# gauravchak/two_tower_models

Hardware: AMD Instinct MI355X
Metric: user-item pairs/sec (in-batch softmax train step: fwd + zero_grad + bwd + dense-exact Adam) (higher is better)
Workload: dtype f32

## Files before the change

### include/tt_hotpath.h

```cpp
#ifndef TT_HOTPATH_H
#define TT_HOTPATH_H

#include <stdint.h>

#ifdef __cplusplus
extern "C" {
#endif

#define TT_ABI_VERSION 6

#define TT_E_BADARG (-1)
#define TT_E_WORKSPACE (-2)
#define TT_E_UNSUPPORTED (-3)

typedef void* tt_stream_t;

int tt_abi_version(void);
const char* tt_last_error_string(void);

int tt_profile_enable(int on);
int tt_profile_read(const char* kernel, double* total_ms, int64_t* launches);
int tt_profile_filter(const char* kernels);
int tt_profile_pause(int paused);

// ... 192 lines not shown
} tt_adam_stash_job;
typedef struct {
  float *W, *M, *V;
  int64_t n_rows, dim;
  const tt_grad_sources* src;
  int64_t n_ids;
  const int32_t *sorted_ids, *perm, *seg_begin, *n_unique;
  void* side;
  int64_t side_bytes;
} tt_adam_finish_job;
int tt_adam_begin_ids(double* hyper, float* tab, int64_t tab_steps, const tt_adam_stash_job* jobs, int32_t n_jobs,
                      tt_stream_t stream);
int tt_adam_tables_finish(const tt_adam_finish_job* jobs, int32_t n_jobs, const double* hyper, tt_stream_t stream);
int tt_adam_begin_ids_planes(double* hyper, float* tab, int64_t tab_steps, const tt_adam_stash_job* jobs, int32_t n_jobs,
                             int32_t planes, tt_stream_t stream);

int tt_stream_create_low_priority(void** out_stream);
int tt_stream_destroy(void* stream);

int tt_adam_advance_tab(double* hyper, float* tab, int64_t tab_steps, tt_stream_t stream);
int tt_adam_rows_catchup(float* W, float* M, float* V, int64_t n_rows, int64_t dim, const int64_t* ids,
                         int64_t n_ids, int32_t* last_step, const double* hyper, const float* tab,
                         int64_t tab_steps, tt_stream_t stream);
int tt_adam_table_lazy(float* W, float* M, float* V, int64_t n_rows, int64_t dim, const double* hyper,
                       const tt_grad_sources* src , int64_t n_ids, const int32_t* sorted_ids,
                       const int32_t* perm, const int32_t* seg_begin, const int32_t* n_unique, void* ws,
                       int64_t ws_bytes, int32_t* last_step, const float* tab, int64_t tab_steps,
                       tt_stream_t stream);
int tt_adam_table_flush(float* W, float* M, float* V, int64_t n_rows, int64_t dim, int32_t* last_step,
                        const double* hyper, const float* tab, int64_t tab_steps, tt_stream_t stream);
// ... 161 lines not shown
```

### two_tower_models_amd/_native.py

```python
from __future__ import annotations

import ctypes as C
import os
from typing import Optional

import torch

_PKG = os.path.dirname(os.path.abspath(__file__))
LIB_PATH = os.path.join(_PKG, "lib", "libtt_hotpath.so")

TT_GEMM_NT, TT_GEMM_NN, TT_GEMM_TN = 0, 1, 2
TT_EPI_NONE, TT_EPI_RELU, TT_EPI_RELU_MASK = 0, 1, 2
TT_F32, TT_BF16, TT_F16X2 = 0, 1, 2
TT_E_BADARG, TT_E_WORKSPACE, TT_E_UNSUPPORTED = -1, -2, -3
TT_DEBIAS_COMBINED, TT_DEBIAS_POSITION, TT_DEBIAS_USER = 0, 1, 2
TT_COMM_ID_BYTES = 128
TT_COMM_F32, TT_COMM_I32, TT_COMM_I64, TT_COMM_U8 = 0, 1, 2, 3
TT_COMM_SUM, TT_COMM_MAX = 0, 1
TT_MAX_GRAD_SOURCES = 4
ABI_VERSION = 6

_vp, _i64, _i32, _int = C.c_void_p, C.c_int64, C.c_int32, C.c_int


class GradSources(C.Structure):

    _fields_ = [
        ("rows", _vp * TT_MAX_GRAD_SOURCES),
        ("ld", _i64 * TT_MAX_GRAD_SOURCES),
        ("first", _i64 * (TT_MAX_GRAD_SOURCES + 1)),
        ("n_sources", _i32),
    ]


class AdamTensor(C.Structure):

    _fields_ = [("p", _vp), ("g", _vp), ("m", _vp), ("v", _vp), ("n", _i64)]


class AdamStashJob(C.Structure):

    _fields_ = [("W", _vp), ("M", _vp), ("V", _vp), ("n_rows", _i64), ("dim", _i64), ("ids", _vp), ("n_ids", _i64),
                ("side", _vp), ("side_bytes", _i64)]


class AdamFinishJob(C.Structure):

    _fields_ = [("W", _vp), ("M", _vp), ("V", _vp), ("n_rows", _i64), ("dim", _i64), ("src", C.POINTER(GradSources)),
                ("n_ids", _i64), ("sorted_ids", _vp), ("perm", _vp), ("seg_begin", _vp), ("n_unique", _vp), ("side", _vp),
                ("side_bytes", _i64)]


# ... 94 lines not shown
    "tt_rowgrad_workspace_bytes": (_i64, [_i64]),
    "tt_rowgrad_plan": (_int, [_vp, _i64, _i64, _vp, _vp, _vp, _vp, _vp, _vp, _i64, _vp]),
    "tt_rowgrad_dense": (_int, [C.POINTER(GradSources), _i64, _i64, _vp, _vp, _vp, _vp, _vp, _vp]),
    "tt_adam_advance": (_int, [_vp, _vp]),
    "tt_adam_table_workspace_bytes": (_i64, [_i64, _i64]),
    "tt_adam_table": (_int, [_vp, _vp, _vp, _i64, _i64, _vp, C.POINTER(GradSources), _i64, _vp, _vp, _vp,
                             _vp, _vp, _i64, _vp]),
    "tt_adam_table_stash": (_int, [_vp, _vp, _vp, _i64, _i64, _i64, _vp, _vp, _vp, _vp, _vp, _i64, _vp]),
    "tt_adam_table_stash_ids": (_int, [_vp, _vp, _vp, _i64, _i64, _vp, _i64, _vp, _i64, _vp]),
    "tt_adam_table_sweep": (_int, [_vp, _vp, _vp, _i64, _i64, _vp, _vp]),
    "tt_adam_tables_sweep": (_int, [C.POINTER(AdamTensor), _i32, _vp, _i32, _vp]),
    "tt_adam_marks_words": (_i64, [_i64]),
    "tt_adam_marked_supported": (_int, [_i64]),
    "tt_adam_mark_rows": (_int, [_vp, _i64, _i64, _vp, _i64, _vp]),
    "tt_adam_tables_sweep_marked": (_int, [C.POINTER(AdamTensor), C.POINTER(_i64), C.POINTER(_vp), _i32, _vp, _i32, _vp]),
    "tt_adam_table_finish": (_int, [_vp, _vp, _vp, _i64, _i64, _vp, C.POINTER(GradSources), _i64, _vp, _vp, _vp,
                                    _vp, _vp, _i64, _vp]),
    "tt_adam_advance_tab": (_int, [_vp, _vp, _i64, _vp]),
    "tt_adam_rows_catchup": (_int, [_vp, _vp, _vp, _i64, _i64, _vp, _i64, _vp, _vp, _vp, _i64, _vp]),
    "tt_adam_table_lazy": (_int, [_vp, _vp, _vp, _i64, _i64, _vp, C.POINTER(GradSources), _i64, _vp, _vp, _vp, _vp,
                                  _vp, _i64, _vp, _vp, _i64, _vp]),
    "tt_adam_table_flush": (_int, [_vp, _vp, _vp, _i64, _i64, _vp, _vp, _vp, _i64, _vp]),
    "tt_stream_create_low_priority": (_int, [C.POINTER(_vp)]),
    "tt_stream_destroy": (_int, [_vp]),
    "tt_adam_dense": (_int, [C.POINTER(AdamTensor), _i32, _vp, _vp]),
    "tt_pack_grads": (_int, [C.POINTER(AdamTensor), _i32, _vp]),
    "tt_copy_buffers": (_int, [C.POINTER(AdamTensor), _i32, _vp]),
    "tt_hist_embed_pool": (_int, [_vp, _i64, _i64, _vp, _i64, _i64, _vp, _vp, _vp, _i64, _vp, _vp]),
    "tt_hist_dx_pool_bwd": (_int, [_vp, _vp, _i64, _i64, _i64, _vp, _i64, _vp, _vp]),
    "tt_hist_pool_bwd": (_int, [_vp, _i64, _i64, _i64, _vp, _i64, _vp]),
# ... 214 lines not shown
```

### two_tower_models_amd/csrc/adam.hip

```cpp
#include <stdlib.h>

#include "common.hpp"

namespace tt {

constexpr int SWEEP_MAX_TABLES_DECL = 4;

constexpr int SWEEP_DEFAULT_PERSIST = 3;

struct AdamConst {
  float one_minus_b1, b2, one_minus_b2, eps, neg_step_size, inv_bc2_sqrt;
};

__device__ __forceinline__ AdamConst load_hyper(const double* __restrict__ h) {
  AdamConst c;
  c.one_minus_b1 = (float)(1.0 - h[1]);
  c.b2 = (float)h[2];
  c.one_minus_b2 = (float)(1.0 - h[2]);
  c.eps = (float)h[3];
  c.neg_step_size = (float)(-h[5]);
  c.inv_bc2_sqrt = (float)(1.0 / h[6]);
  return c;
}

// ... 20 lines not shown
  al = e - (ah - p);
}
__device__ __forceinline__ double pow_steps(double b, double step) {
  double rh = 1.0, rl = 0.0, bh = b, bl = 0.0;
  for (unsigned long long e = (unsigned long long)step; e; e >>= 1) {
    if (e & 1) dd_mul(rh, rl, bh, bl);
    dd_mul(bh, bl, bh, bl);
  }
  return rh;
}
__device__ __forceinline__ void step_consts_from_doubles(double lr, double b1, double b2, double step,
                                                         double& h5, double& h6) {
  h5 = lr / (1.0 - pow_steps(b1, step));
  h6 = sqrt(1.0 - pow_steps(b2, step));
}
__global__ void adam_advance_kernel(double* h, float* tab, int64_t tab_cap) {
  const double step = h[4] + 1.0;
  h[4] = step;
  step_consts_from_doubles(h[0], h[1], h[2], step, h[5], h[6]);
  const int64_t j = (int64_t)step;
  if (tab && j < tab_cap) {
    tab[2 * j] = (float)(-h[5]);
    tab[2 * j + 1] = (float)(1.0 / h[6]);
  }
}

__device__ __forceinline__ const float* source_row(const tt_grad_sources& s, int64_t pos) {
  int k = 0;
#pragma unroll
  for (int q = 1; q < TT_MAX_GRAD_SOURCES; ++q)
    if (q < s.n_sources && pos >= s.first[q]) k = q;
  return s.rows[k] + (pos - s.first[k]) * s.ld[k];
}

template <bool FROM_SIDE>
__global__ __launch_bounds__(256) void adam_touched_kernel(const float* __restrict__ W, const float* __restrict__ M,
                                                           const float* __restrict__ V, int64_t n_rows, int64_t dim,
                                                           const double* __restrict__ hyper, const tt_grad_sources src,
                                                           const int32_t* __restrict__ sorted_ids,
                                                           const int32_t* __restrict__ perm,
// ... 97 lines not shown

struct StashJobs {
  const float* W[SWEEP_MAX_TABLES_DECL];
  const float* M[SWEEP_MAX_TABLES_DECL];
  const float* V[SWEEP_MAX_TABLES_DECL];
  const int64_t* ids[SWEEP_MAX_TABLES_DECL];
  float* side[SWEEP_MAX_TABLES_DECL];
  int64_t n_rows[SWEEP_MAX_TABLES_DECL], dim[SWEEP_MAX_TABLES_DECL], n_ids[SWEEP_MAX_TABLES_DECL];
  unsigned first_block[SWEEP_MAX_TABLES_DECL + 1];
  int n;
};
__global__ __launch_bounds__(256) void adam_begin_ids_kernel(const StashJobs jobs, double* h, float* tab, int64_t tab_cap, int planes,
                                                             int advance) {
  const unsigned n_stash = jobs.first_block[jobs.n];
  if (blockIdx.x == n_stash) {
    if (threadIdx.x == 0 && advance) {
      const double step = h[4] + 1.0;
      h[4] = step;
      step_consts_from_doubles(h[0], h[1], h[2], step, h[5], h[6]);
      const int64_t j = (int64_t)step;
      if (tab && j < tab_cap) {
        tab[2 * j] = (float)(-h[5]);
        tab[2 * j + 1] = (float)(1.0 / h[6]);
      }
    }
    return;
  }
  int t = 0;
#pragma unroll
  for (int q = 1; q < SWEEP_MAX_TABLES_DECL; ++q)
    if (q < jobs.n && blockIdx.x >= jobs.first_block[q]) t = q;
  adam_stash_ids_body(jobs.W[t], jobs.M[t], jobs.V[t], jobs.n_rows[t], jobs.dim[t], jobs.ids[t], jobs.n_ids[t], jobs.side[t],
                      blockIdx.x - jobs.first_block[t], planes);
}

__global__ __launch_bounds__(256) void adam_writeback_kernel(float* __restrict__ W, float* __restrict__ M,
                                                             float* __restrict__ V, int64_t n_rows, int64_t dim,
                                                             const int32_t* __restrict__ sorted_ids,
                                                             const int32_t* __restrict__ seg_begin,
                                                             const int32_t* __restrict__ perm,
// ... 137 lines not shown
      ctr[1] = 0;
      __threadfence();
    }
  }
}

constexpr int SWEEP_MAX_TABLES = SWEEP_MAX_TABLES_DECL;
struct SweepTables {
  float4* W[SWEEP_MAX_TABLES];
  float4* M[SWEEP_MAX_TABLES];
  float4* V[SWEEP_MAX_TABLES];
  int64_t n4[SWEEP_MAX_TABLES];
  unsigned first_chunk[SWEEP_MAX_TABLES + 1];
  int n;
};
template <int ITERS, int UNR>
__global__ __launch_bounds__(256) void adam_sweep_tables_kernel(const SweepTables tabs, const double* __restrict__ hyper,
                                                                unsigned* __restrict__ ctr) {
  const AdamConst c = load_hyper(hyper);
  const unsigned n_chunks = tabs.first_chunk[tabs.n];
  __shared__ unsigned s_next[2];
  if (threadIdx.x == 0) s_next[0] = atomicAdd(&ctr[0], 1u);
  __syncthreads();
  unsigned ch = s_next[0];
  int par = 0;
  while (ch < n_chunks) {
    if (threadIdx.x == 0) s_next[par ^ 1] = atomicAdd(&ctr[0], 1u);
    int t = 0;
#pragma unroll
    for (int q = 1; q < SWEEP_MAX_TABLES; ++q)
      if (q < tabs.n && ch >= tabs.first_chunk[q]) t = q;
    float4* __restrict__ W = tabs.W[t];
    float4* __restrict__ M = tabs.M[t];
    float4* __restrict__ V = tabs.V[t];
    const int64_t n4 = tabs.n4[t];
    const int64_t base = (int64_t)(ch - tabs.first_chunk[t]) * (256 * ITERS) + threadIdx.x;
#pragma unroll UNR
    for (int k = 0; k < ITERS; ++k) {
      const int64_t i = base + (int64_t)k * 256;
      if (i >= n4) break;
      float4 p = sweep_load(W + i), m = sweep_load(M + i), v = sweep_load(V + i);
      adam_elem_zero_grad(p.x, m.x, v.x, c);
      adam_elem_zero_grad(p.y, m.y, v.y, c);
      adam_elem_zero_grad(p.z, m.z, v.z, c);
      adam_elem_zero_grad(p.w, m.w, v.w, c);
      sweep_store(p, W + i); sweep_store(m, M + i); sweep_store(v, V + i);
    }
    __syncthreads();
    par ^= 1;
    ch = s_next[par];
  }
  if (threadIdx.x == 0) {
    if (atomicAdd(&ctr[1], 1u) == gridDim.x - 1) {
      ctr[0] = 0;
      ctr[1] = 0;
      __threadfence();
    }
  }
}

struct SweepTablesMarked {
  SweepTables t;
  const unsigned* marks[SWEEP_MAX_TABLES];
  int sh[SWEEP_MAX_TABLES];
};
template <int ITERS, int PAIR>
__global__ __launch_bounds__(256) void adam_sweep_tables_marked_kernel(const SweepTablesMarked tm, const double* __restrict__ hyper,
                                                                       unsigned* __restrict__ ctr) {
  const AdamConst c = load_hyper(hyper);
  const unsigned n_chunks = tm.t.first_chunk[tm.t.n];
  __shared__ unsigned s_next[2];
  if (threadIdx.x == 0) s_next[0] = atomicAdd(&ctr[0], 1u);
  __syncthreads();
  unsigned ch = s_next[0];
  int par = 0;
  while (ch < n_chunks) {
    if (threadIdx.x == 0) s_next[par ^ 1] = atomicAdd(&ctr[0], 1u);
    const unsigned chu = __builtin_amdgcn_readfirstlane(ch);
    int t = 0;
#pragma unroll
    for (int q = 1; q < SWEEP_MAX_TABLES; ++q)
      if (q < tm.t.n && chu >= tm.t.first_chunk[q]) t = q;
    float4* __restrict__ W = tm.t.W[t];
    float4* __restrict__ M = tm.t.M[t];
    float4* __restrict__ V = tm.t.V[t];
    const int64_t n4 = tm.t.n4[t];
    const unsigned lc = chu - tm.t.first_chunk[t];
    const int sh = tm.sh[t];
    const int64_t r0 = (int64_t)lc * ((256 * ITERS) >> sh);
    const unsigned* __restrict__ mk = tm.marks[t];
    unsigned w0 = 0, w1 = 0, w2 = 0, w3 = 0;
    if (mk) {
      const unsigned* mw = mk + (r0 >> 5);
      w0 = mw[0]; w1 = mw[1]; w2 = mw[2]; w3 = mw[3];
    }
    const int64_t base = (int64_t)lc * (256 * ITERS) + threadIdx.x;
#pragma unroll
    for (int k = 0; k < ITERS; k += PAIR) {
      float4 p[PAIR], m[PAIR], v[PAIR];
      bool live[PAIR];
#pragma unroll
      for (int q = 0; q < PAIR; ++q) {
        const int64_t i = base + (int64_t)(k + q) * 256;
        const int64_t row = r0 + (((k + q) * 256 + (int)threadIdx.x) >> sh);
        const int wj = (int)((row >> 5) - (r0 >> 5));
        const unsigned word = wj == 0 ? w0 : wj == 1 ? w1 : wj == 2 ? w2 : w3;
        live[q] = i < n4 && !((word >> (row & 31)) & 1u);
      }
#pragma unroll
      for (int q = 0; q < PAIR; ++q) {
        const int64_t i = base + (int64_t)(k + q) * 256;
        if (live[q]) { p[q] = sweep_load(W + i); m[q] = sweep_load(M + i); v[q] = sweep_load(V + i); }
      }
#pragma unroll
      for (int q = 0; q < PAIR; ++q) {
        const int64_t i = base + (int64_t)(k + q) * 256;
        if (live[q]) {
          adam_elem_zero_grad(p[q].x, m[q].x, v[q].x, c);
          adam_elem_zero_grad(p[q].y, m[q].y, v[q].y, c);
          adam_elem_zero_grad(p[q].z, m[q].z, v[q].z, c);
          adam_elem_zero_grad(p[q].w, m[q].w, v[q].w, c);
          sweep_store(p[q], W + i); sweep_store(m[q], M + i); sweep_store(v[q], V + i);
        }
      }
    }
    __syncthreads();
    par ^= 1;
    ch = s_next[par];
  }
  if (threadIdx.x == 0) {
    if (atomicAdd(&ctr[1], 1u) == gridDim.x - 1) {
      ctr[0] = 0;
      ctr[1] = 0;
      __threadfence();
    }
  }
}

__global__ __launch_bounds__(256) void adam_mark_rows_kernel(const int64_t* __restrict__ ids, int64_t n_ids, int64_t n_rows,
                                                             unsigned* __restrict__ marks) {
  const int64_t i = (int64_t)blockIdx.x * 256 + threadIdx.x;
  if (i >= n_ids) return;
  const int64_t row = ids[i];
  if (row >= 0 && row < n_rows) atomicOr(&marks[row >> 5], 1u << (row & 31));
}

__global__ __launch_bounds__(256) void adam_sweep_scalar_kernel(float* __restrict__ W, float* __restrict__ M,
                                                                float* __restrict__ V, int64_t i0, int64_t n,
                                                                const double* __restrict__ hyper) {
  const AdamConst c = load_hyper(hyper);
  const int64_t stride = (int64_t)gridDim.x * blockDim.x;
  for (int64_t i = i0 + (int64_t)blockIdx.x * blockDim.x + threadIdx.x; i < n; i += stride) {
    float p = W[i], m = M[i], v = V[i];
    adam_elem_zero_grad(p, m, v, c);
    W[i] = p; M[i] = m; V[i] = v;
  }
}

__device__ __forceinline__ void replay_consts(AdamConst& c, const double* __restrict__ h, const float* __restrict__ tab,
// ... 350 lines not shown
  if (!ids || !marks) return fail_arg("tt_adam_mark_rows: null pointer");
  if (n_ids <= 0 || n_rows <= 0) return fail_arg("tt_adam_mark_rows: sizes");
  if (marks_words < tt_adam_marks_words(n_rows)) { set_error("tt_adam_mark_rows: bitmap of %lld words < %lld", (long long)marks_words, (long long)tt_adam_marks_words(n_rows)); return TT_E_WORKSPACE; }
  hipStream_t st = S(stream);
  hipError_t e = hipMemsetAsync(marks, 0, (size_t)marks_words * 4, st);
  if (e != hipSuccess) { set_error("tt_adam_mark_rows: hipMemsetAsync: %s", hipGetErrorString(e)); return (int)e; }
  adam_mark_rows_kernel<<<(unsigned)ceil_div(n_ids, 256), 256, 0, st>>>(ids, n_ids, n_rows, marks);
  return check_launch("adam_mark_rows_kernel");
}

extern "C" int tt_adam_marked_supported(int64_t dim) {
  if (dim < 32 || dim > 4096 || (dim & (dim - 1))) return 0;
  return 1;
}

extern "C" int tt_adam_tables_sweep_marked(const tt_adam_tensor* tables, const int64_t* dims, const uint32_t* const* marks,
                                           int32_t n_tables, const double* hyper, int32_t n_wgs, tt_stream_t stream) {
  if (!tables || !dims || !marks || !hyper) return fail_arg("tt_adam_tables_sweep_marked: null pointer");
  if (n_tables <= 0 || n_tables > SWEEP_MAX_TABLES) return fail_arg("tt_adam_tables_sweep_marked: 1..4 tables");
  SweepTablesMarked tm{};
  unsigned chunks = 0;
  for (int t = 0; t < n_tables; ++t) {
    const tt_adam_tensor& d = tables[t];
    if (!d.p || !d.m || !d.v || d.n <= 0) return fail_arg("tt_adam_tables_sweep_marked: descriptor");
    if (!tt_adam_marked_supported(dims[t]) || d.n % dims[t]) return fail_arg("tt_adam_tables_sweep_marked: dim must be a power of two in [32, 4096]");
    if ((reinterpret_cast<uintptr_t>(d.p) | reinterpret_cast<uintptr_t>(d.m) | reinterpret_cast<uintptr_t>(d.v)) & 15)
      return fail_arg("tt_adam_tables_sweep_marked: 16-byte aligned tables");
    tm.t.W[t] = reinterpret_cast<float4*>(d.p); tm.t.M[t] = reinterpret_cast<float4*>(d.m); tm.t.V[t] = reinterpret_cast<float4*>(d.v);
    tm.t.n4[t] = d.n / 4;
    tm.t.first_chunk[t] = chunks;
    const int64_t c = ceil_div(d.n / 4, 256 * 4);
    if (c + chunks >= (1ll << 32)) return fail_arg("tt_adam_tables_sweep_marked: too many chunks");
    chunks += (unsigned)c;
    tm.marks[t] = marks[t];
    int sh = 0;
    while ((4ll << sh) < dims[t]) ++sh;
    tm.sh[t] = sh;
  }
  tm.t.first_chunk[n_tables] = chunks;
  tm.t.n = n_tables;
  static const int wgs_env = getenv("TT_SWEEP_WGS") ? atoi(getenv("TT_SWEEP_WGS")) : 0;
  const int want = getenv("TT_SWEEP_WGS") ? wgs_env : n_wgs;
  unsigned* ctr = reinterpret_cast<unsigned*>(const_cast<double*>(hyper) + 7);
  unsigned grid = (unsigned)(device_cu_count() * SWEEP_DEFAULT_PERSIST);
  if (want > 0 && (unsigned)want < grid) grid = (unsigned)want;
  hipStream_t st = S(stream);
  ProfScope prof("adam_sweep_kernel", st);
  adam_sweep_tables_marked_kernel<4, 2><<<grid, 256, 0, st>>>(tm, hyper, ctr);
  return check_launch("adam_sweep_tables_marked_kernel");
}

extern "C" int tt_stream_create_low_priority(void** out) {
  if (!out) return fail_arg("tt_stream_create_low_priority: null pointer");
  int least = 0, greatest = 0;
  hipError_t e = hipDeviceGetStreamPriorityRange(&least, &greatest);
  if (e != hipSuccess) { set_error("hipDeviceGetStreamPriorityRange: %s", hipGetErrorString(e)); return (int)e; }
  hipStream_t s;
  e = hipStreamCreateWithPriority(&s, hipStreamNonBlocking, least);
  if (e != hipSuccess) { set_error("hipStreamCreateWithPriority: %s", hipGetErrorString(e)); return (int)e; }
  *out = reinterpret_cast<void*>(s);
  return 0;
}
extern "C" int tt_stream_destroy(void* stream) {
  if (!stream) return 0;
// ... 230 lines not shown
```

### two_tower_models_amd/optim.py

```python
from __future__ import annotations

import ctypes as C
import os
import weakref
from typing import Dict, Iterable, List, Optional, Sequence

import torch

from . import _native as N
from . import ops
from .sweep_controller import GroupSweepController, SweepController


_RELEASE_AT_LOGITS = True
_TAB_MIN_STEPS = 1 << 16
_SPLIT_MIN_IDS = 65536
_MARK_ROWS = True
_HOLD_SWEEP = True


class _TableStep:

    __slots__ = ("plan", "side", "announced", "marked", "n_rows")

# ... 61 lines not shown
        self.capture_overlap = False
        self._sweep_ctl = (GroupSweepController(self._group_reduce(self._sharded[0]))
                           if self._sharded and self._sharded[0]._tt_shard.world > 1 else SweepController())
        self._plan_stream: Optional[torch.cuda.Stream] = None
        self._plan_done: Optional[torch.cuda.Event] = None
        self._plans_pending = False
        self._plan_ready: Optional[torch.cuda.Event] = None
        self._begun: Optional[Dict[torch.nn.Parameter, _TableStep]] = None
        self._sweep_done: Optional[torch.cuda.Event] = None
        self._side_bufs: Dict[int, torch.Tensor] = {}
        self._marks: Dict[int, torch.Tensor] = {}
        self._sweep_pending = None
        self._sweep_pending_marked = False
        self._sweep_events = None
        self._catchup_last: Dict[int, tuple] = {}

    def _init_state(self) -> None:
        dev = N.require_device(*self._params)
        g = self.param_groups[0]
        self._hyper = torch.tensor([g["lr"], g["betas"][0], g["betas"][1], g["eps"], 0.0, 0.0, 0.0, 0.0],
                                   dtype=torch.float64, device=dev)
        arena = bool(self._tables) and all(p.is_cuda for p in self._tables) and os.environ.get("TT_ADAM_NO_ARENA") is None
        in_arena = {id(p) for p in self._tables} if arena else set()
        for p in self._params:
            if p.dtype != torch.float32 or not p.is_contiguous():
                raise TypeError("DenseExactAdam needs contiguous fp32 parameters")
            st = self.state[p]
            for key in ("exp_avg", "exp_avg_sq"):
                if key not in st and id(p) in in_arena:
                    continue
# ... 156 lines not shown
    def state_dict(self):
        self.flush()
        sd = super().state_dict()
        step = torch.tensor(float(self.step_count))
        for st in sd["state"].values():
            st["step"] = step.clone()
        return sd

    def load_state_dict(self, state_dict) -> None:
        super().load_state_dict(state_dict)
        steps = {int(float(st["step"])) for st in self.state.values() if "step" in st}
        if len(steps) > 1:
            raise ValueError("DenseExactAdam needs one common step count for all parameters")
        self._resume_step = self._sweep_ctl.resume_step = steps.pop() if steps else 0
        self._begun = None
        self._ready = False

    def _advance_lazy(self) -> None:
        if (self._host_steps + 2 >= self._tab_steps and not self._tab_pinned
                and not torch.cuda.is_current_stream_capturing()):
            bigger = torch.zeros(4 * self._tab_steps, dtype=torch.float32, device=self._tab.device)
            bigger[: 2 * self._tab_steps].copy_(self._tab)
            self._tab, self._tab_steps = bigger, 2 * self._tab_steps
        N.check(N.load().tt_adam_advance_tab(self._hyper.data_ptr(), self._tab.data_ptr(), self._tab_steps,
                                             N.stream()), "tt_adam_advance_tab")
        self._host_steps += 1

    @property
    def step_count(self) -> int:
        if not self._ready:
# ... 1 lines not shown
        return int(self._hyper[4].item())

    def _side(self, p: torch.Tensor, nbytes: int) -> torch.Tensor:
        buf = self._side_bufs.get(id(p))
        if buf is None or buf.numel() < nbytes:
            buf = torch.empty(int(nbytes * 1.25) + 256, dtype=torch.uint8, device=p.device)
            self._side_bufs[id(p)] = buf
        return buf

    def _begin_overlapped(self, announced: Optional[Dict[int, Sequence[torch.Tensor]]] = None, hold_sweep: bool = False) -> None:
        lib = N.load()
        if not self._ready:
            self._init_state()
        hyper = self._hyper.data_ptr()
        capturing = torch.cuda.is_current_stream_capturing()
        ev_begin = None
        if capturing:
            self._sweep_ctl.record = None
        else:
            self._tune_sweep()
            ev_begin = torch.cuda.Event(enable_timing=True)
            ev_begin.record()
            self._sweep_ctl.began(ev_begin, self._host_steps + 1)
        if announced is None:
            N.check(lib.tt_adam_advance(hyper, N.stream()), "tt_adam_advance")
        self._host_steps += 1
        begun: Dict[torch.nn.Parameter, _TableStep] = {}
        stash_jobs = []
        todo = []
        for p in self._tables:
            blocks = announced.get(id(p)) if announced is not None else p._tt_lookups
            if not blocks:
                continue
            shard = getattr(p, "_tt_shard", None)
            n_rows = p.shape[0] if shard is None else shard.n_local
            if n_rows > 0:
                todo.append((p, blocks, n_rows))
        n_stashed = sum(sum(b.numel() for b in blocks) for _, blocks, _ in todo)
        split_planes = announced is not None and not capturing and 0 < len(todo) <= 4 and n_stashed >= _SPLIT_MIN_IDS
        marked = (split_planes and _MARK_ROWS and all(lib.tt_adam_marked_supported(p.shape[1]) for p, _, _ in todo)
                  and all((p.data_ptr() | self.state[p]["exp_avg"].data_ptr() | self.state[p]["exp_avg_sq"].data_ptr()) % 16 == 0
                          for p, _, _ in todo))
        for p, blocks, n_rows in todo:
            dim = p.shape[1]
            shard = getattr(p, "_tt_shard", None)
            st = self.state[p]
            plan = ops.RowPlan(blocks, n_rows + (1 if shard is not None else 0), slot=f"plan{id(p)}", defer=announced is not None)
            side = None if marked else self._side(p, lib.tt_adam_table_workspace_bytes(plan.n, dim))
            if marked:
                if shard is None:
                    p._tt_active = ops.ActiveMarks(plan.block_sizes)
            elif announced is not None:
                stash_jobs.append((p.data_ptr(), st["exp_avg"].data_ptr(), st["exp_avg_sq"].data_ptr(), n_rows, dim,
                                   plan.ids.data_ptr(), plan.n, side.data_ptr(), side.numel()))
                if shard is None:
                    p_plane = side[: plan.n * dim * 4].view(torch.float32).view(plan.n, dim)
                    p._tt_active = ops.ActiveStash(p_plane, plan.block_sizes)
            else:
                N.check(lib.tt_adam_table_stash(p.data_ptr(), st["exp_avg"].data_ptr(), st["exp_avg_sq"].data_ptr(),
                                                n_rows, dim, plan.n, plan.sorted_ids.data_ptr(), plan.perm.data_ptr(),
                                                plan.seg_begin.data_ptr(), plan.n_unique.data_ptr(), side.data_ptr(),
                                                side.numel(), N.stream()), "tt_adam_table_stash")
            begun[p] = _TableStep(plan, side, announced is not None, marked, n_rows)
        if marked:
            N.check(lib.tt_adam_advance(hyper, N.stream()), "tt_adam_advance")
        elif announced is not None:
            jobs = (N.AdamStashJob * max(len(stash_jobs), 1))()
            for i, j in enumerate(stash_jobs):
                (jobs[i].W, jobs[i].M, jobs[i].V, jobs[i].n_rows, jobs[i].dim, jobs[i].ids, jobs[i].n_ids, jobs[i].side,
                 jobs[i].side_bytes) = j
            if split_planes:
                N.check(lib.tt_adam_begin_ids_planes(hyper, None, 0, jobs, len(stash_jobs), 1, N.stream()), "tt_adam_begin_ids_planes")
            else:
                N.check(lib.tt_adam_begin_ids(hyper, None, 0, jobs, len(stash_jobs), N.stream()), "tt_adam_begin_ids")
        main = torch.cuda.current_stream()
        ready = torch.cuda.Event()
        ready.record(main)

# ... 36 lines not shown
                if mark_ptrs is not None:
                    dims = (C.c_int64 * len(begun))(*[p.shape[1] for p in begun])
                    N.check(lib.tt_adam_tables_sweep_marked(descs, dims, mark_ptrs, len(begun), hyper, self._sweep_wgs,
                                                            self._side_stream.cuda_stream), "tt_adam_tables_sweep_marked")
                else:
                    N.check(lib.tt_adam_tables_sweep(descs, len(begun), hyper, self._sweep_wgs, self._side_stream.cuda_stream),
                            "tt_adam_tables_sweep")
            self._sweep_done = torch.cuda.Event(enable_timing=not capturing)
            self._sweep_done.record(self._side_stream)
            if not capturing:
                self._sweep_ctl.swept(ev_s0, self._sweep_done)
            if self._sweep_events is not None and ev_s0 is not None and len(self._sweep_events) < 65536:
                self._sweep_events.append((ev_s0, self._sweep_done))

        self._sweep_done = None
        n_announced = sum(ts.plan.n for ts in begun.values()) if announced is not None else 0
        if _HOLD_SWEEP and announced is not None and not capturing and ((n_announced >= 65536 and not self._sharded) or hold_sweep):
            self._sweep_pending = launch_sweep
            self._sweep_pending_marked = marked
            self._hold_for_logits = bool(hold_sweep) and _RELEASE_AT_LOGITS
            if self._hold_for_logits:
                ops.held_sweeps.add(self)
        else:
            self._sweep_pending = None
            launch_sweep()
        self._plan_done = None
        self._plans_pending = announced is not None and bool(begun)
        self._plan_ready = ready if self._plans_pending else None
        self._begun = begun

    def keep_sweep_events(self, on: bool = True) -> None:
        self._sweep_events = [] if on else None

    def sweep_launch_ms(self):
        total, n = 0.0, 0
        for a, b in self._sweep_events or ():
            b.synchronize()
            total += a.elapsed_time(b)
            n += 1
        return total, n

    def held_sweep_is_marked(self) -> bool:
        return getattr(self, "_sweep_pending", None) is not None and bool(getattr(self, "_sweep_pending_marked", False))
# ... 120 lines not shown
    @staticmethod
    def _ordered_rows(p) -> List[torch.Tensor]:
        blocks = p._tt_rowgrads
        if len(blocks) != len(p._tt_lookups) or any(b.index is None for b in blocks):
            raise RuntimeError(
                "a table lookup of the last forward received no gradient (or more than one forward ran "
                "before zero_grad()); use DenseExactAdam(..., overlap_sweep=False) for this call pattern")
        return [b.rows for b in sorted(blocks, key=lambda b: b.index)]

    @torch.no_grad()
    def step(self, closure=None):
        if closure is not None:
            raise NotImplementedError("closure is not supported")
        if not self._ready:
            self._init_state()
        lib = N.load()
        hyper = self._hyper.data_ptr()
        if self._sharded and self._begun is None:
            raise RuntimeError("row-sharded tables: step() without a train_forward that announced its lookups (the models' "
                               "train_forward does; a custom forward must call model._announce_lookups first)")
        reduce = self._start_dense_allreduce() if self._sharded else None
        self.release_sweep()
        if self._begun is not None:
            self._launch_plans(side=False)
            torch.cuda.current_stream().wait_event(self._sweep_done)
            if self._plan_done is not None:
                torch.cuda.current_stream().wait_event(self._plan_done)
                self._plan_done = None
            if self._begun:
                jobs = (N.AdamFinishJob * len(self._begun))()
                for i, (p, ts) in enumerate(self._begun.items()):
                    st = self.state[p]
                    ts.plan.attach(self._ordered_rows(p))
                    j = jobs[i]
                    j.W, j.M, j.V = p.data_ptr(), st["exp_avg"].data_ptr(), st["exp_avg_sq"].data_ptr()
                    shard = getattr(p, "_tt_shard", None)
                    j.n_rows = p.shape[0] if shard is None else shard.n_local
                    j.dim, j.src, j.n_ids = p.shape[1], C.pointer(ts.plan.sources), ts.plan.n
                    j.sorted_ids, j.perm = ts.plan.sorted_ids.data_ptr(), ts.plan.perm.data_ptr()
                    j.seg_begin, j.n_unique = ts.plan.seg_begin.data_ptr(), ts.plan.n_unique.data_ptr()
                    j.side, j.side_bytes = (None, 0) if ts.marked else (ts.side.data_ptr(), ts.side.numel())
                N.check(lib.tt_adam_tables_finish(jobs, len(self._begun), hyper, N.stream()), "tt_adam_tables_finish")
            self._begun = None
            if self._sweep_ctl.record is not None:
                end = torch.cuda.Event(enable_timing=True)
                end.record()
                self._sweep_ctl.ended(end)
        elif self.lazy:
            if self._prefetch_done is not None:
                torch.cuda.current_stream().wait_event(self._prefetch_done)
                self._prefetch_done, self._prefetch_keep = None, None
            self._catchup_last.clear()
            self._advance_lazy()
            todo = []
            for p in self._tables:
                blocks = p._tt_rowgrads
                if p.grad is not None:
                    raise RuntimeError("embedding table received a dense gradient while in row-gradient mode")
                if not blocks:
                    continue
                if all(b.index is not None for b in blocks):
# ... 40 lines not shown
        if reduce is not None:
            self._finish_dense_allreduce(reduce, lib, hyper)
            return None
        live = [p for p in self._dense if p.grad is not None]
        if live:
            descs = (N.AdamTensor * len(live))()
            keep = []
            for i, p in enumerate(live):
                gr = p.grad if p.grad.is_contiguous() else p.grad.contiguous()
                keep.append(gr)
                st = self.state[p]
                descs[i].p, descs[i].g = p.data_ptr(), gr.data_ptr()
                descs[i].m, descs[i].v = st["exp_avg"].data_ptr(), st["exp_avg_sq"].data_ptr()
                descs[i].n = p.numel()
            N.check(lib.tt_adam_dense(descs, len(live), hyper, N.stream()), "tt_adam_dense")
        return None
```

Before: 1.514 million.

## Chain marked Adam table sweep on side stream across optimizer step boundary

Adds a chained mode in which a fused mark+advance kernel runs on a side stream, followed by a marked sweep that skips touched rows. The main stream no longer waits for the sweep before the table finish step; it only waits at the very end of step(). Double-buffered mark bitmaps are cleared a step ahead, and an alone-flag lets surplus sweep workgroups exit once the main stream reaches the end of step, so the sweep can overlap backward and dense Adam without keeping the whole GPU. This adds cross-stream ordering complexity and a possible race on marks and hyper state.

```diff
diff --git a/include/tt_hotpath.h b/include/tt_hotpath.h
--- a/include/tt_hotpath.h
+++ b/include/tt_hotpath.h
@@ -230,6 +230,17 @@
 int tt_adam_tables_finish(const tt_adam_finish_job* jobs, int32_t n_jobs, const double* hyper, tt_stream_t stream);
 int tt_adam_begin_ids_planes(double* hyper, float* tab, int64_t tab_steps, const tt_adam_stash_job* jobs, int32_t n_jobs,
                              int32_t planes, tt_stream_t stream);
+typedef struct {
+  const int64_t* ids;
+  int64_t n_ids, n_rows;
+  uint32_t* marks;
+  int64_t marks_words;
+} tt_adam_mark_job;
+int tt_adam_mark_advance(double* hyper, const tt_adam_mark_job* jobs , int32_t n_jobs, tt_stream_t stream);
+int tt_adam_tables_sweep_chained(const struct tt_adam_tensor_s* tables , const int64_t* dims ,
+                                 const uint32_t* const* marks , int32_t n_tables,
+                                 const double* hyper, int32_t n_wgs, int32_t alone_wgs, const uint32_t* alone_flag,
+                                 uint32_t tag, tt_stream_t stream);
 
 int tt_stream_create_low_priority(void** out_stream);
 int tt_stream_destroy(void* stream);
diff --git a/two_tower_models_amd/_native.py b/two_tower_models_amd/_native.py
--- a/two_tower_models_amd/_native.py
+++ b/two_tower_models_amd/_native.py
@@ -36,6 +36,11 @@
 class AdamTensor(C.Structure):
 
     _fields_ = [("p", _vp), ("g", _vp), ("m", _vp), ("v", _vp), ("n", _i64)]
+
+
+class AdamMarkJob(C.Structure):
+
+    _fields_ = [("ids", _vp), ("n_ids", _i64), ("n_rows", _i64), ("marks", _vp), ("marks_words", _i64)]
 
 
 class AdamStashJob(C.Structure):
@@ -160,6 +165,9 @@
     "tt_adam_marked_supported": (_int, [_i64]),
     "tt_adam_mark_rows": (_int, [_vp, _i64, _i64, _vp, _i64, _vp]),
     "tt_adam_tables_sweep_marked": (_int, [C.POINTER(AdamTensor), C.POINTER(_i64), C.POINTER(_vp), _i32, _vp, _i32, _vp]),
+    "tt_adam_mark_advance": (_int, [_vp, C.POINTER(AdamMarkJob), _i32, _vp]),
+    "tt_adam_tables_sweep_chained": (_int, [C.POINTER(AdamTensor), C.POINTER(_i64), C.POINTER(_vp), _i32, _vp, _i32, _i32, _vp,
+                                            C.c_uint32, _vp]),
     "tt_adam_table_finish": (_int, [_vp, _vp, _vp, _i64, _i64, _vp, C.POINTER(GradSources), _i64, _vp, _vp, _vp,
                                     _vp, _vp, _i64, _vp]),
     "tt_adam_advance_tab": (_int, [_vp, _vp, _i64, _vp]),
diff --git a/two_tower_models_amd/csrc/adam.hip b/two_tower_models_amd/csrc/adam.hip
--- a/two_tower_models_amd/csrc/adam.hip
+++ b/two_tower_models_amd/csrc/adam.hip
@@ -1,4 +1,6 @@
 #include <stdlib.h>
+
+#include <type_traits>
 
 #include "common.hpp"
 
@@ -58,7 +60,7 @@
   h5 = lr / (1.0 - pow_steps(b1, step));
   h6 = sqrt(1.0 - pow_steps(b2, step));
 }
-__global__ void adam_advance_kernel(double* h, float* tab, int64_t tab_cap) {
+__device__ __forceinline__ void advance_step(double* h, float* tab, int64_t tab_cap) {
   const double step = h[4] + 1.0;
   h[4] = step;
   step_consts_from_doubles(h[0], h[1], h[2], step, h[5], h[6]);
@@ -68,6 +70,7 @@
     tab[2 * j + 1] = (float)(1.0 / h[6]);
   }
 }
+__global__ void adam_advance_kernel(double* h, float* tab, int64_t tab_cap) { advance_step(h, tab, tab_cap); }
 
 __device__ __forceinline__ const float* source_row(const tt_grad_sources& s, int64_t pos) {
   int k = 0;
@@ -195,16 +198,7 @@
                                                              int advance) {
   const unsigned n_stash = jobs.first_block[jobs.n];
   if (blockIdx.x == n_stash) {
-    if (threadIdx.x == 0 && advance) {
-      const double step = h[4] + 1.0;
-      h[4] = step;
-      step_consts_from_doubles(h[0], h[1], h[2], step, h[5], h[6]);
-      const int64_t j = (int64_t)step;
-      if (tab && j < tab_cap) {
-        tab[2 * j] = (float)(-h[5]);
-        tab[2 * j + 1] = (float)(1.0 / h[6]);
-      }
-    }
+    if (threadIdx.x == 0 && advance) advance_step(h, tab, tab_cap);
     return;
   }
   int t = 0;
@@ -372,37 +366,69 @@
   unsigned first_chunk[SWEEP_MAX_TABLES + 1];
   int n;
 };
-template <int ITERS, int UNR>
-__global__ __launch_bounds__(256) void adam_sweep_tables_kernel(const SweepTables tabs, const double* __restrict__ hyper,
-                                                                unsigned* __restrict__ ctr) {
+struct SweepTablesMarked {
+  SweepTables t;
+  const unsigned* marks[SWEEP_MAX_TABLES];
+  int sh[SWEEP_MAX_TABLES];
+};
+struct SweepTablesChained {
+  SweepTablesMarked m;
+  const unsigned* alone_flag;
+  unsigned tag, alone_wgs;
+};
+constexpr unsigned SWEEP_NO_CHUNK = 0xffffffffu;
+__device__ __forceinline__ unsigned next_chunk_or_leave(const SweepTablesChained& a, unsigned* ctr) {
+  if (a.alone_flag && blockIdx.x >= a.alone_wgs &&
+      __hip_atomic_load(a.alone_flag, __ATOMIC_RELAXED, __HIP_MEMORY_SCOPE_AGENT) == a.tag)
+    return SWEEP_NO_CHUNK;
+  return atomicAdd(&ctr[0], 1u);
+}
+template <int ITERS, int PAIR>
+__device__ __forceinline__ void sweep_chunk_marked(const SweepTablesMarked& tm, unsigned chu, const AdamConst& c);
+
+template <int ITERS, int UNR, bool MARKS = false>
+__global__ __launch_bounds__(256) void adam_sweep_tables_kernel(const std::conditional_t<MARKS, SweepTablesChained, SweepTables> tabs,
+                                                                const double* __restrict__ hyper, unsigned* __restrict__ ctr) {
   const AdamConst c = load_hyper(hyper);
-  const unsigned n_chunks = tabs.first_chunk[tabs.n];
+  unsigned n_chunks;
+  if constexpr (MARKS) n_chunks = tabs.m.t.first_chunk[tabs.m.t.n];
+  else n_chunks = tabs.first_chunk[tabs.n];
   __shared__ unsigned s_next[2];
-  if (threadIdx.x == 0) s_next[0] = atomicAdd(&ctr[0], 1u);
+  if (threadIdx.x == 0) {
+    if constexpr (MARKS) s_next[0] = next_chunk_or_leave(tabs, ctr);
+    else s_next[0] = atomicAdd(&ctr[0], 1u);
+  }
   __syncthreads();
   unsigned ch = s_next[0];
   int par = 0;
   while (ch < n_chunks) {
-    if (threadIdx.x == 0) s_next[par ^ 1] = atomicAdd(&ctr[0], 1u);
-    int t = 0;
-#pragma unroll
-    for (int q = 1; q < SWEEP_MAX_TABLES; ++q)
-      if (q < tabs.n && ch >= tabs.first_chunk[q]) t = q;
-    float4* __restrict__ W = tabs.W[t];
-    float4* __restrict__ M = tabs.M[t];
-    float4* __restrict__ V = tabs.V[t];
-    const int64_t n4 = tabs.n4[t];
-    const int64_t base = (int64_t)(ch - tabs.first_chunk[t]) * (256 * ITERS) + threadIdx.x;
+    if (threadIdx.x == 0) {
+      if constexpr (MARKS) s_next[par ^ 1] = next_chunk_or_leave(tabs, ctr);
+      else s_next[par ^ 1] = atomicAdd(&ctr[0], 1u);
+    }
+    if constexpr (MARKS) {
+      sweep_chunk_marked<ITERS, UNR>(tabs.m, __builtin_amdgcn_readfirstlane(ch), c);
+    } else {
+      int t = 0;
+#pragma unroll
+      for (int q = 1; q < SWEEP_MAX_TABLES; ++q)
+        if (q < tabs.n && ch >= tabs.first_chunk[q]) t = q;
+      float4* __restrict__ W = tabs.W[t];
+      float4* __restrict__ M = tabs.M[t];
+      float4* __restrict__ V = tabs.V[t];
+      const int64_t n4 = tabs.n4[t];
+      const int64_t base = (int64_t)(ch - tabs.first_chunk[t]) * (256 * ITERS) + threadIdx.x;
 #pragma unroll UNR
-    for (int k = 0; k < ITERS; ++k) {
-      const int64_t i = base + (int64_t)k * 256;
-      if (i >= n4) break;
-      float4 p = sweep_load(W + i), m = sweep_load(M + i), v = sweep_load(V + i);
-      adam_elem_zero_grad(p.x, m.x, v.x, c);
-      adam_elem_zero_grad(p.y, m.y, v.y, c);
-      adam_elem_zero_grad(p.z, m.z, v.z, c);
-      adam_elem_zero_grad(p.w, m.w, v.w, c);
-      sweep_store(p, W + i); sweep_store(m, M + i); sweep_store(v, V + i);
+      for (int k = 0; k < ITERS; ++k) {
+        const int64_t i = base + (int64_t)k * 256;
+        if (i >= n4) break;
+        float4 p = sweep_load(W + i), m = sweep_load(M + i), v = sweep_load(V + i);
+        adam_elem_zero_grad(p.x, m.x, v.x, c);
+        adam_elem_zero_grad(p.y, m.y, v.y, c);
+        adam_elem_zero_grad(p.z, m.z, v.z, c);
+        adam_elem_zero_grad(p.w, m.w, v.w, c);
+        sweep_store(p, W + i); sweep_store(m, M + i); sweep_store(v, V + i);
+      }
     }
     __syncthreads();
     par ^= 1;
@@ -417,11 +443,56 @@
   }
 }
 
-struct SweepTablesMarked {
-  SweepTables t;
-  const unsigned* marks[SWEEP_MAX_TABLES];
-  int sh[SWEEP_MAX_TABLES];
-};
+template <int ITERS, int PAIR>
+__device__ __forceinline__ void sweep_chunk_marked(const SweepTablesMarked& tm, unsigned chu, const AdamConst& c) {
+  int t = 0;
+#pragma unroll
+  for (int q = 1; q < SWEEP_MAX_TABLES; ++q)
+    if (q < tm.t.n && chu >= tm.t.first_chunk[q]) t = q;
+  float4* __restrict__ W = tm.t.W[t];
+  float4* __restrict__ M = tm.t.M[t];
+  float4* __restrict__ V = tm.t.V[t];
+  const int64_t n4 = tm.t.n4[t];
+  const unsigned lc = chu - tm.t.first_chunk[t];
+  const int sh = tm.sh[t];
+  const int64_t r0 = (int64_t)lc * ((256 * ITERS) >> sh);
+  const unsigned* __restrict__ mk = tm.marks[t];
+  unsigned w0 = 0, w1 = 0, w2 = 0, w3 = 0;
+  if (mk) {
+    const unsigned* mw = mk + (r0 >> 5);
+    w0 = mw[0]; w1 = mw[1]; w2 = mw[2]; w3 = mw[3];
+  }
+  const int64_t base = (int64_t)lc * (256 * ITERS) + threadIdx.x;
+#pragma unroll
+  for (int k = 0; k < ITERS; k += PAIR) {
+    float4 p[PAIR], m[PAIR], v[PAIR];
+    bool live[PAIR];
+#pragma unroll
+    for (int q = 0; q < PAIR; ++q) {
+      const int64_t i = base + (int64_t)(k + q) * 256;
+      const int64_t row = r0 + (((k + q) * 256 + (int)threadIdx.x) >> sh);
+      const int wj = (int)((row >> 5) - (r0 >> 5));
+      const unsigned word = wj == 0 ? w0 : wj == 1 ? w1 : wj == 2 ? w2 : w3;
+      live[q] = i < n4 && !((word >> (row & 31)) & 1u);
+    }
+#pragma unroll
+    for (int q = 0; q < PAIR; ++q) {
+      const int64_t i = base + (int64_t)(k + q) * 256;
+      if (live[q]) { p[q] = sweep_load(W + i); m[q] = sweep_load(M + i); v[q] = sweep_load(V + i); }
+    }
+#pragma unroll
+    for (int q = 0; q < PAIR; ++q) {
+      const int64_t i = base + (int64_t)(k + q) * 256;
+      if (live[q]) {
+        adam_elem_zero_grad(p[q].x, m[q].x, v[q].x, c);
+        adam_elem_zero_grad(p[q].y, m[q].y, v[q].y, c);
+        adam_elem_zero_grad(p[q].z, m[q].z, v[q].z, c);
+        adam_elem_zero_grad(p[q].w, m[q].w, v[q].w, c);
+        sweep_store(p[q], W + i); sweep_store(m[q], M + i); sweep_store(v[q], V + i);
+      }
+    }
+  }
+}
 template <int ITERS, int PAIR>
 __global__ __launch_bounds__(256) void adam_sweep_tables_marked_kernel(const SweepTablesMarked tm, const double* __restrict__ hyper,
                                                                        unsigned* __restrict__ ctr) {
@@ -434,54 +505,7 @@
   int par = 0;
   while (ch < n_chunks) {
     if (threadIdx.x == 0) s_next[par ^ 1] = atomicAdd(&ctr[0], 1u);
-    const unsigned chu = __builtin_amdgcn_readfirstlane(ch);
-    int t = 0;
-#pragma unroll
-    for (int q = 1; q < SWEEP_MAX_TABLES; ++q)
-      if (q < tm.t.n && chu >= tm.t.first_chunk[q]) t = q;
-    float4* __restrict__ W = tm.t.W[t];
-    float4* __restrict__ M = tm.t.M[t];
-    float4* __restrict__ V = tm.t.V[t];
-    const int64_t n4 = tm.t.n4[t];
-    const unsigned lc = chu - tm.t.first_chunk[t];
-    const int sh = tm.sh[t];
-    const int64_t r0 = (int64_t)lc * ((256 * ITERS) >> sh);
-    const unsigned* __restrict__ mk = tm.marks[t];
-    unsigned w0 = 0, w1 = 0, w2 = 0, w3 = 0;
-    if (mk) {
-      const unsigned* mw = mk + (r0 >> 5);
-      w0 = mw[0]; w1 = mw[1]; w2 = mw[2]; w3 = mw[3];
-    }
-    const int64_t base = (int64_t)lc * (256 * ITERS) + threadIdx.x;
-#pragma unroll
-    for (int k = 0; k < ITERS; k += PAIR) {
-      float4 p[PAIR], m[PAIR], v[PAIR];
-      bool live[PAIR];
-#pragma unroll
-      for (int q = 0; q < PAIR; ++q) {
-        const int64_t i = base + (int64_t)(k + q) * 256;
-        const int64_t row = r0 + (((k + q) * 256 + (int)threadIdx.x) >> sh);
-        const int wj = (int)((row >> 5) - (r0 >> 5));
-        const unsigned word = wj == 0 ? w0 : wj == 1 ? w1 : wj == 2 ? w2 : w3;
-        live[q] = i < n4 && !((word >> (row & 31)) & 1u);
-      }
-#pragma unroll
-      for (int q = 0; q < PAIR; ++q) {
-        const int64_t i = base + (int64_t)(k + q) * 256;
-        if (live[q]) { p[q] = sweep_load(W + i); m[q] = sweep_load(M + i); v[q] = sweep_load(V + i); }
-      }
-#pragma unroll
-      for (int q = 0; q < PAIR; ++q) {
-        const int64_t i = base + (int64_t)(k + q) * 256;
-        if (live[q]) {
-          adam_elem_zero_grad(p[q].x, m[q].x, v[q].x, c);
-          adam_elem_zero_grad(p[q].y, m[q].y, v[q].y, c);
-          adam_elem_zero_grad(p[q].z, m[q].z, v[q].z, c);
-          adam_elem_zero_grad(p[q].w, m[q].w, v[q].w, c);
-          sweep_store(p[q], W + i); sweep_store(m[q], M + i); sweep_store(v[q], V + i);
-        }
-      }
-    }
+    sweep_chunk_marked<ITERS, PAIR>(tm, __builtin_amdgcn_readfirstlane(ch), c);
     __syncthreads();
     par ^= 1;
     ch = s_next[par];
@@ -501,6 +525,28 @@
   if (i >= n_ids) return;
   const int64_t row = ids[i];
   if (row >= 0 && row < n_rows) atomicOr(&marks[row >> 5], 1u << (row & 31));
+}
+
+struct MarkJobs {
+  const int64_t* ids[SWEEP_MAX_TABLES_DECL];
+  int64_t n_ids[SWEEP_MAX_TABLES_DECL], n_rows[SWEEP_MAX_TABLES_DECL];
+  unsigned* marks[SWEEP_MAX_TABLES_DECL];
+  unsigned first_block[SWEEP_MAX_TABLES_DECL + 1];
+  int n;
+};
+__global__ __launch_bounds__(256) void adam_mark_advance_kernel(const MarkJobs jobs, double* h) {
+  if (blockIdx.x == jobs.first_block[jobs.n]) {
+    if (threadIdx.x == 0) advance_step(h, nullptr, 0);
+    return;
+  }
+  int t = 0;
+#pragma unroll
+  for (int q = 1; q < SWEEP_MAX_TABLES_DECL; ++q)
+    if (q < jobs.n && blockIdx.x >= jobs.first_block[q]) t = q;
+  const int64_t i = (int64_t)(blockIdx.x - jobs.first_block[t]) * 256 + threadIdx.x;
+  if (i >= jobs.n_ids[t]) return;
+  const int64_t row = jobs.ids[t][i];
+  if (row >= 0 && row < jobs.n_rows[t]) atomicOr(&jobs.marks[t][row >> 5], 1u << (row & 31));
 }
 
 __global__ __launch_bounds__(256) void adam_sweep_scalar_kernel(float* __restrict__ W, float* __restrict__ M,
@@ -881,11 +927,10 @@
   return 1;
 }
 
-extern "C" int tt_adam_tables_sweep_marked(const tt_adam_tensor* tables, const int64_t* dims, const uint32_t* const* marks,
-                                           int32_t n_tables, const double* hyper, int32_t n_wgs, tt_stream_t stream) {
+static int fill_marked_tables(const tt_adam_tensor* tables, const int64_t* dims, const uint32_t* const* marks, int32_t n_tables,
+                              const double* hyper, SweepTablesMarked& tm) {
   if (!tables || !dims || !marks || !hyper) return fail_arg("tt_adam_tables_sweep_marked: null pointer");
   if (n_tables <= 0 || n_tables > SWEEP_MAX_TABLES) return fail_arg("tt_adam_tables_sweep_marked: 1..4 tables");
-  SweepTablesMarked tm{};
   unsigned chunks = 0;
   for (int t = 0; t < n_tables; ++t) {
     const tt_adam_tensor& d = tables[t];
@@ -897,7 +942,7 @@
     tm.t.n4[t] = d.n / 4;
     tm.t.first_chunk[t] = chunks;
     const int64_t c = ceil_div(d.n / 4, 256 * 4);
-    if (c + chunks >= (1ll << 32)) return fail_arg("tt_adam_tables_sweep_marked: too many chunks");
+    if (c + chunks >= (1ll << 32) - 1) return fail_arg("tt_adam_tables_sweep_marked: too many chunks");
     chunks += (unsigned)c;
     tm.marks[t] = marks[t];
     int sh = 0;
@@ -906,15 +951,66 @@
   }
   tm.t.first_chunk[n_tables] = chunks;
   tm.t.n = n_tables;
+  return 0;
+}
+
+static unsigned sweep_grid(int32_t n_wgs) {
   static const int wgs_env = getenv("TT_SWEEP_WGS") ? atoi(getenv("TT_SWEEP_WGS")) : 0;
   const int want = getenv("TT_SWEEP_WGS") ? wgs_env : n_wgs;
-  unsigned* ctr = reinterpret_cast<unsigned*>(const_cast<double*>(hyper) + 7);
   unsigned grid = (unsigned)(device_cu_count() * SWEEP_DEFAULT_PERSIST);
   if (want > 0 && (unsigned)want < grid) grid = (unsigned)want;
+  return grid;
+}
+
+extern "C" int tt_adam_tables_sweep_marked(const tt_adam_tensor* tables, const int64_t* dims, const uint32_t* const* marks,
+                                           int32_t n_tables, const double* hyper, int32_t n_wgs, tt_stream_t stream) {
+  SweepTablesMarked tm{};
+  int rc = fill_marked_tables(tables, dims, marks, n_tables, hyper, tm);
+  if (rc) return rc;
+  unsigned* ctr = reinterpret_cast<unsigned*>(const_cast<double*>(hyper) + 7);
+  const unsigned grid = sweep_grid(n_wgs);
   hipStream_t st = S(stream);
   ProfScope prof("adam_sweep_kernel", st);
   adam_sweep_tables_marked_kernel<4, 2><<<grid, 256, 0, st>>>(tm, hyper, ctr);
   return check_launch("adam_sweep_tables_marked_kernel");
+}
+
+extern "C" int tt_adam_tables_sweep_chained(const tt_adam_tensor* tables, const int64_t* dims, const uint32_t* const* marks,
+                                            int32_t n_tables, const double* hyper, int32_t n_wgs, int32_t alone_wgs,
+                                            const uint32_t* alone_flag, uint32_t tag, tt_stream_t stream) {
+  SweepTablesChained a{};
+  int rc = fill_marked_tables(tables, dims, marks, n_tables, hyper, a.m);
+  if (rc) return rc;
+  unsigned* ctr = reinterpret_cast<unsigned*>(const_cast<double*>(hyper) + 7);
+  const unsigned grid = sweep_grid(n_wgs);
+  const bool thin = alone_flag && alone_wgs > 0 && (unsigned)alone_wgs < grid;
+  a.alone_flag = thin ? alone_flag : nullptr;
+  a.tag = tag;
+  a.alone_wgs = thin ? (unsigned)alone_wgs : grid;
+  hipStream_t st = S(stream);
+  ProfScope prof("adam_sweep_kernel", st);
+  adam_sweep_tables_kernel<4, 2, true><<<grid, 256, 0, st>>>(a, hyper, ctr);
+  return check_launch("adam_sweep_tables_kernel");
+}
+
+extern "C" int tt_adam_mark_advance(double* hyper, const tt_adam_mark_job* jobs, int32_t n_jobs, tt_stream_t stream) {
+  if (!hyper || (n_jobs > 0 && !jobs)) return fail_arg("tt_adam_mark_advance: null pointer");
+  if (n_jobs < 0 || n_jobs > SWEEP_MAX_TABLES) return fail_arg("tt_adam_mark_advance: 0..4 tables");
+  MarkJobs a{};
+  a.n = n_jobs;
+  unsigned blocks = 0;
+  for (int i = 0; i < n_jobs; ++i) {
+    const tt_adam_mark_job& j = jobs[i];
+    if (!j.ids || !j.marks) return fail_arg("tt_adam_mark_advance: null pointer");
+    if (j.n_ids <= 0 || j.n_rows <= 0 || ceil_div(j.n_ids, 256) + blocks >= (1ll << 31)) return fail_arg("tt_adam_mark_advance: sizes");
+    if (j.marks_words < tt_adam_marks_words(j.n_rows)) { set_error("tt_adam_mark_advance: bitmap of %lld words < %lld", (long long)j.marks_words, (long long)tt_adam_marks_words(j.n_rows)); return TT_E_WORKSPACE; }
+    a.ids[i] = j.ids; a.n_ids[i] = j.n_ids; a.n_rows[i] = j.n_rows; a.marks[i] = j.marks;
+    a.first_block[i] = blocks;
+    blocks += (unsigned)ceil_div(j.n_ids, 256);
+  }
+  for (int i = n_jobs; i <= SWEEP_MAX_TABLES; ++i) a.first_block[i] = blocks;
+  adam_mark_advance_kernel<<<blocks + 1, 256, 0, S(stream)>>>(a, hyper);
+  return check_launch("adam_mark_advance_kernel");
 }
 
 extern "C" int tt_stream_create_low_priority(void** out) {
diff --git a/two_tower_models_amd/optim.py b/two_tower_models_amd/optim.py
--- a/two_tower_models_amd/optim.py
+++ b/two_tower_models_amd/optim.py
@@ -99,6 +99,13 @@
         self._sweep_pending_marked = False
         self._sweep_events = None
         self._catchup_last: Dict[int, tuple] = {}
+        self._chained = False
+        self._chain_last_done: Optional[torch.cuda.Event] = None
+        self._chain_main_done = None
+        self._chain_cleared = None
+        self._chain_marks: Dict[tuple, torch.Tensor] = {}
+        self._alone_flag: Optional[torch.Tensor] = None
+        self._alone_tag: Optional[int] = None
 
     def _init_state(self) -> None:
         dev = N.require_device(*self._params)
@@ -285,6 +292,7 @@
             raise ValueError("DenseExactAdam needs one common step count for all parameters")
         self._resume_step = self._sweep_ctl.resume_step = steps.pop() if steps else 0
         self._begun = None
+        self._chained, self._chain_last_done = False, None
         self._ready = False
 
     def _advance_lazy(self) -> None:
@@ -316,17 +324,6 @@
             self._init_state()
         hyper = self._hyper.data_ptr()
         capturing = torch.cuda.is_current_stream_capturing()
-        ev_begin = None
-        if capturing:
-            self._sweep_ctl.record = None
-        else:
-            self._tune_sweep()
-            ev_begin = torch.cuda.Event(enable_timing=True)
-            ev_begin.record()
-            self._sweep_ctl.began(ev_begin, self._host_steps + 1)
-        if announced is None:
-            N.check(lib.tt_adam_advance(hyper, N.stream()), "tt_adam_advance")
-        self._host_steps += 1
         begun: Dict[torch.nn.Parameter, _TableStep] = {}
         stash_jobs = []
         todo = []
@@ -340,9 +337,29 @@
                 todo.append((p, blocks, n_rows))
         n_stashed = sum(sum(b.numel() for b in blocks) for _, blocks, _ in todo)
         split_planes = announced is not None and not capturing and 0 < len(todo) <= 4 and n_stashed >= _SPLIT_MIN_IDS
-        marked = (split_planes and _MARK_ROWS and all(lib.tt_adam_marked_supported(p.shape[1]) for p, _, _ in todo)
-                  and all((p.data_ptr() | self.state[p]["exp_avg"].data_ptr() | self.state[p]["exp_avg_sq"].data_ptr()) % 16 == 0
-                          for p, _, _ in todo))
+        markable = (announced is not None and not capturing and 0 < len(todo) <= 4 and _MARK_ROWS
+                    and all(lib.tt_adam_marked_supported(p.shape[1]) for p, _, _ in todo)
+                    and all((p.data_ptr() | self.state[p]["exp_avg"].data_ptr() | self.state[p]["exp_avg_sq"].data_ptr()) % 16 == 0
+                            for p, _, _ in todo))
+        held = announced is not None and not capturing and ((n_stashed >= 65536 and not self._sharded) or hold_sweep)
+        chained = (markable and not held and not self._sharded and self.overlap_sweep == "forward"
+                   and os.environ.get("TT_ADAM_CHAIN", "1") != "0")
+        marked = chained or (split_planes and markable)
+        self._chained = chained
+        if not chained:
+            self._chain_last_done = None
+        if capturing:
+            self._sweep_ctl.record = None
+        else:
+            self._tune_sweep()
+            ev_begin = self._chain_last_done
+            if ev_begin is None:
+                ev_begin = torch.cuda.Event(enable_timing=True)
+                ev_begin.record()
+            self._sweep_ctl.began(ev_begin, self._host_steps + 1)
+        if announced is None:
+            N.check(lib.tt_adam_advance(hyper, N.stream()), "tt_adam_advance")
+        self._host_steps += 1
         for p, blocks, n_rows in todo:
             dim = p.shape[1]
             shard = getattr(p, "_tt_shard", None)
@@ -364,6 +381,9 @@
                                                 plan.seg_begin.data_ptr(), plan.n_unique.data_ptr(), side.data_ptr(),
                                                 side.numel(), N.stream()), "tt_adam_table_stash")
             begun[p] = _TableStep(plan, side, announced is not None, marked, n_rows)
+        if chained:
+            self._launch_chained(begun)
+            return
         if marked:
             N.check(lib.tt_adam_advance(hyper, N.stream()), "tt_adam_advance")
         elif announced is not None:
@@ -430,8 +450,7 @@
                 self._sweep_events.append((ev_s0, self._sweep_done))
 
         self._sweep_done = None
-        n_announced = sum(ts.plan.n for ts in begun.values()) if announced is not None else 0
-        if _HOLD_SWEEP and announced is not None and not capturing and ((n_announced >= 65536 and not self._sharded) or hold_sweep):
+        if _HOLD_SWEEP and held:
             self._sweep_pending = launch_sweep
             self._sweep_pending_marked = marked
             self._hold_for_logits = bool(hold_sweep) and _RELEASE_AT_LOGITS
@@ -443,6 +462,59 @@
         self._plan_done = None
         self._plans_pending = announced is not None and bool(begun)
         self._plan_ready = ready if self._plans_pending else None
+        self._begun = begun
+
+    def _launch_chained(self, begun: Dict[torch.nn.Parameter, _TableStep]) -> None:
+        lib = N.load()
+        hyper = self._hyper.data_ptr()
+        main, side = torch.cuda.current_stream(), self._side_stream
+        dev = next(iter(begun)).device
+        parity = self._host_steps & 1
+        jobs = (N.AdamMarkJob * len(begun))()
+        mark_ptrs = (C.c_void_p * len(begun))()
+        for i, (p, ts) in enumerate(begun.items()):
+            words = lib.tt_adam_marks_words(ts.n_rows)
+            bm = self._chain_marks.get((id(p), parity))
+            if bm is None or bm.numel() < words:
+                bm = self._chain_marks[(id(p), parity)] = torch.zeros(words, dtype=torch.int32, device=dev)
+            elif self._chain_cleared != (self._host_steps, main):
+                bm.zero_()
+            j = jobs[i]
+            j.ids, j.n_ids, j.n_rows, j.marks, j.marks_words = ts.plan.ids.data_ptr(), ts.plan.n, ts.n_rows, bm.data_ptr(), bm.numel()
+            mark_ptrs[i] = bm.data_ptr()
+        ready = torch.cuda.Event()
+        ready.record(main)
+        if self._chain_main_done is not None and self._chain_main_done[1] != main:
+            side.wait_event(self._chain_main_done[0])
+        side.wait_event(ready)
+        N.check(lib.tt_adam_mark_advance(hyper, jobs, len(begun), side.cuda_stream), "tt_adam_mark_advance")
+        advanced = ev_s0 = torch.cuda.Event(enable_timing=True)
+        advanced.record(side)
+        main.wait_event(advanced)
+        descs = (N.AdamTensor * len(begun))()
+        for i, p in enumerate(begun):
+            st = self.state[p]
+            descs[i].p, descs[i].g, descs[i].m, descs[i].v = p.data_ptr(), None, st["exp_avg"].data_ptr(), st["exp_avg_sq"].data_ptr()
+            descs[i].n = p.numel()
+        dims = (C.c_int64 * len(begun))(*[p.shape[1] for p in begun])
+        alone = os.environ.get("TT_SWEEP_ALONE_WGS")
+        alone = int(alone) if alone is not None else 2 * torch.cuda.get_device_properties(dev).multi_processor_count
+        if self._alone_flag is None:
+            self._alone_flag = torch.zeros(1, dtype=torch.int32, device=dev)
+        self._alone_tag = (self._host_steps & 0x7FFFFFFF) if alone > 0 else None
+        N.check(lib.tt_adam_tables_sweep_chained(descs, dims, mark_ptrs, len(begun), hyper, self._sweep_wgs, max(alone, 0),
+                                                 self._alone_flag.data_ptr(), self._alone_tag or 0, side.cuda_stream),
+                "tt_adam_tables_sweep_chained")
+        self._sweep_done = torch.cuda.Event(enable_timing=True)
+        self._sweep_done.record(side)
+        self._chain_last_done = self._sweep_done
+        self._sweep_ctl.swept(ev_s0, self._sweep_done)
+        if self._sweep_events is not None and len(self._sweep_events) < 65536:
+            self._sweep_events.append((ev_s0, self._sweep_done))
+        self._sweep_pending = None
+        self._plan_done = None
+        self._plans_pending = True
+        self._plan_ready = ready
         self._begun = begun
 
     def keep_sweep_events(self, on: bool = True) -> None:
@@ -593,6 +665,7 @@
             raise NotImplementedError("closure is not supported")
         if not self._ready:
             self._init_state()
+        chained = False
         lib = N.load()
         hyper = self._hyper.data_ptr()
         if self._sharded and self._begun is None:
@@ -602,7 +675,9 @@
         self.release_sweep()
         if self._begun is not None:
             self._launch_plans(side=False)
-            torch.cuda.current_stream().wait_event(self._sweep_done)
+            chained = self._chained
+            if not chained:
+                torch.cuda.current_stream().wait_event(self._sweep_done)
             if self._plan_done is not None:
                 torch.cuda.current_stream().wait_event(self._plan_done)
                 self._plan_done = None
@@ -622,8 +697,9 @@
                 N.check(lib.tt_adam_tables_finish(jobs, len(self._begun), hyper, N.stream()), "tt_adam_tables_finish")
             self._begun = None
             if self._sweep_ctl.record is not None:
-                end = torch.cuda.Event(enable_timing=True)
-                end.record()
+                end = self._sweep_done if chained else torch.cuda.Event(enable_timing=True)
+                if not chained:
+                    end.record()
                 self._sweep_ctl.ended(end)
         elif self.lazy:
             if self._prefetch_done is not None:
@@ -694,4 +770,17 @@
                 descs[i].m, descs[i].v = st["exp_avg"].data_ptr(), st["exp_avg_sq"].data_ptr()
                 descs[i].n = p.numel()
             N.check(lib.tt_adam_dense(descs, len(live), hyper, N.stream()), "tt_adam_dense")
+        if chained:
+            main = torch.cuda.current_stream()
+            for (_, parity), bm in self._chain_marks.items():
+                if parity == (self._host_steps + 1) & 1:
+                    bm.zero_()
+            self._chain_cleared = (self._host_steps + 1, main)
+            done = torch.cuda.Event()
+            done.record(main)
+            self._chain_main_done = (done, main)
+            if self._alone_tag is not None:
+                self._alone_flag.fill_(self._alone_tag)
+            main.wait_event(self._sweep_done)
+            self._chained = False
         return None
```

Measured after the change: 1.540 million, median of 6. 1.02x the previous value.
